# syshin1014/wssdl_bus

Measured on AMD Instinct MI355X. Metric: images/sec (train step, 600x1000), higher is better.
Workload: dtype f32; 1 GPU; resnet50_joint_b8; backbone=ResNet-50, image=600x1000, images_per_gpu=8, supervised_per_gpu=4, weak_per_gpu=4, mode=joint, parallelism=image-parallel dp1, RCCL grad all-reduce, sampling_rng=device, fused_rpn_softmax=True, padded_rois=False, miopen_find=True, miopen_find_db=wssdl_bus_amd/miopen_db (HIP.3_5_0_20250912-42-1199-g2584e35062), miopen_searched=True

## Files before the change

### wssdl_bus_amd/build.py

```python
import os
import subprocess
import sys

HERE = os.path.dirname(os.path.abspath(__file__))
CSRC = os.path.join(HERE, "csrc")
OUT = os.environ.get("WSSDL_BUS_HIP_LIB") or os.path.join(HERE, "libwssdl_bus_hip.so")
SOURCES = ["api_common.hip", "bbox_overlaps.hip", "nms.hip", "proposal.hip", "anchor_target.hip",
           "roi_targets.hip", "roi_pool.hip", "roi_pool_compact.hip", "roi_pool_blocks.hip", "roi_pool_walk.hip", "mil.hip", "image.hip", "loss.hip",
           "post_detect.hip", "order_sort.hip"]
HEADERS = ["common.hip.h", "nms.hip.h", "select.hip.h", "order_sort.hip.h", "roi_pool.hip.h", os.path.join("..", "..", "include", "wssdl_bus_hip.h")]
FLAGS = ["-O3", "-std=c++17", "--offload-arch=gfx950", "-ffp-contract=off", "-fPIC", "-shared",
         "-fvisibility=hidden", "-Wall", "-Wno-unused-function"]


def hipcc():
    for c in (os.environ.get("HIPCC"), "/opt/rocm/bin/hipcc", "hipcc"):
        if c and (os.path.isabs(c) and os.path.exists(c) or not os.path.isabs(c)):
            return c
    return "hipcc"


def is_stale():
    if not os.path.exists(OUT):
        return True
    t = os.path.getmtime(OUT)
    deps = [os.path.join(CSRC, s) for s in SOURCES + HEADERS] + [os.path.abspath(__file__), os.path.join(HERE, "isa_check.py")]
    return any(os.path.getmtime(d) > t for d in deps)


def _digest(paths, extra=""):
    import hashlib
    h = hashlib.sha256(extra.encode())
    for q in paths:
        with open(q, "rb") as f:
            h.update(f.read())
    return h.hexdigest()[:16]


def _compile_one(args):
    src, obj, flags, verbose = args
    tmp = "%s.%d.tmp" % (obj, os.getpid())
    cmd = [hipcc()] + flags + ["-c", src, "-o", tmp]
    if verbose:
        print("[wssdl_bus_amd] " + " ".join(cmd), flush=True)
    subprocess.check_call(cmd)
    os.replace(tmp, obj)
    return obj


def compile_objects(sources, headers, flags, verbose=True, jobs=None):
    from concurrent.futures import ThreadPoolExecutor
    objdir = os.path.join(CSRC, "_obj")
    os.makedirs(objdir, exist_ok=True)
    cflags = [f for f in flags if f != "-shared"]
    hdrs = [os.path.join(CSRC, h) for h in headers]
    todo, objs = [], []
    for s in sources:
        src = os.path.join(CSRC, s)
        tag = _digest([src] + hdrs, " ".join(cflags))
        obj = os.path.join(objdir, "%s.%s.o" % (os.path.basename(s), tag))
        objs.append(obj)
        if not os.path.exists(obj):
            for old in os.listdir(objdir):
                if old.startswith(os.path.basename(s) + "."):
                    os.remove(os.path.join(objdir, old))
            todo.append((src, obj, cflags, verbose))
    jobs = jobs or int(os.environ.get("WSSDL_BUILD_JOBS", "0")) or min(8, os.cpu_count() or 1)
    with ThreadPoolExecutor(max_workers=max(1, jobs)) as ex:
        list(ex.map(_compile_one, todo))
    return objs


def build(force=False, verbose=True):
    if not force and not is_stale():
        return OUT
    if force:
        import shutil
        shutil.rmtree(os.path.join(CSRC, "_obj"), ignore_errors=True)
    objs = compile_objects(SOURCES, HEADERS, FLAGS, verbose)
    tmp = "%s.%d.tmp" % (OUT, os.getpid())
    cmd = [hipcc(), "-shared", "-fPIC", "--offload-arch=gfx950", "-fvisibility=hidden"] + objs + ["-o", tmp]
    if verbose:
        print("[wssdl_bus_amd] " + " ".join(cmd))
    subprocess.check_call(cmd)
    from . import isa_check
    try:
        isa_check.check_library(tmp)
    except Exception:
        os.remove(tmp)
        raise
    os.replace(tmp, OUT)
    return OUT


PLUMB_OUT = os.path.join(HERE, "libwssdl_plumbing_hip.so")
PLUMB_SOURCES = [os.path.join("plumbing", "rowbn.hip"), os.path.join("plumbing", "im2col.hip")]
PLUMB_FLAGS = ["-O3", "-std=c++17", "--offload-arch=gfx950", "-fPIC", "-shared", "-fvisibility=hidden",
               "-Wall"]


def build_plumbing(force=False, verbose=True):
    srcs = [os.path.join(CSRC, s) for s in PLUMB_SOURCES]
    if not force and os.path.exists(PLUMB_OUT) and \
            all(os.path.getmtime(f) <= os.path.getmtime(PLUMB_OUT) for f in srcs + [os.path.abspath(__file__)]):
        return PLUMB_OUT
    tmp = "%s.%d.tmp" % (PLUMB_OUT, os.getpid())
    cmd = [hipcc()] + PLUMB_FLAGS + srcs + ["-o", tmp]
    if verbose:
        print("[wssdl_bus_amd] " + " ".join(cmd))
    subprocess.check_call(cmd)
    os.replace(tmp, PLUMB_OUT)
    return PLUMB_OUT


if __name__ == "__main__":
    build(force="--force" in sys.argv)
    build_plumbing(force="--force" in sys.argv)
    print(OUT)
    print(PLUMB_OUT)
```

### wssdl_bus_amd/csrc/plumbing/rowbn.hip

```cpp
#include <hip/hip_runtime.h>
#include <stdint.h>

#define PLUMB_API extern "C" __attribute__((visibility("default")))

namespace {

constexpr int BLOCK = 256;
constexpr int MAX_PARTIAL_BLOCKS = 1024;

typedef float float4v __attribute__((ext_vector_type(4)));

template <int MODE, bool RELU, bool MASKED>
__global__ __launch_bounds__(BLOCK) void rowbn_partial_kernel(
    const float *__restrict__ x, const float *__restrict__ dy, const float *__restrict__ scale,
    const float *__restrict__ shift, long long M, int C, long long rows_per_block,
    double *__restrict__ partial, const float *__restrict__ mask, int per) {
    __shared__ double red[BLOCK][8];
    const int C4 = C >> 2;
    const int L = C4 < BLOCK ? C4 : BLOCK;
    const int RS = BLOCK / L;
    const int t = threadIdx.x;
    const int lc = t % L, lr = t / L;
    const long long r0 = (long long)blockIdx.x * rows_per_block;
    const long long r1 = r0 + rows_per_block < M ? r0 + rows_per_block : M;
    double *out = partial + (size_t)blockIdx.x * 2 * C;
    for (int cc = 0; cc * L < C4; ++cc) {
        const int c4 = cc * L + lc;
        double s[4] = {0, 0, 0, 0}, q[4] = {0, 0, 0, 0};
        float4v sc = {0, 0, 0, 0}, sh = {0, 0, 0, 0};
        if (MODE == 1 && RELU) {
            sc = reinterpret_cast<const float4v *>(scale)[c4];
            sh = reinterpret_cast<const float4v *>(shift)[c4];
        }
        if (lr < RS) {
            long long r = r0 + lr;
            for (; r + RS < r1; r += 2 * RS) {
                bool live0 = true, live1 = true;
                if (MASKED) {
                    live0 = mask[(unsigned)r / (unsigned)per] != 0.0f;
                    live1 = mask[(unsigned)(r + RS) / (unsigned)per] != 0.0f;
                    if (!live0 && !live1) continue;
                }
                const float4v zero4 = {0, 0, 0, 0};
                const float4v a0 = live0 ? reinterpret_cast<const float4v *>(x + (size_t)r * C)[c4] : zero4;
                const float4v a1 = live1 ? reinterpret_cast<const float4v *>(x + (size_t)(r + RS) * C)[c4] : zero4;
                float4v g0, g1;
                if (MODE == 1) {
                    g0 = live0 ? reinterpret_cast<const float4v *>(dy + (size_t)r * C)[c4] : zero4;
                    g1 = live1 ? reinterpret_cast<const float4v *>(dy + (size_t)(r + RS) * C)[c4] : zero4;
                }
#pragma unroll
                for (int j = 0; j < 4; ++j) {
                    if (MODE == 0) {
                        s[j] += (double)a0[j] + (double)a1[j];
                        q[j] += (double)a0[j] * (double)a0[j] + (double)a1[j] * (double)a1[j];
                    } else {
                        float u0 = g0[j], u1 = g1[j];
                        if (RELU) {
                            if (!(a0[j] * sc[j] + sh[j] > 0.0f)) u0 = 0.0f;
                            if (!(a1[j] * sc[j] + sh[j] > 0.0f)) u1 = 0.0f;
                        }
                        if (MASKED) {
                            if (!live0) u0 = 0.0f;
                            if (!live1) u1 = 0.0f;
                        }
                        s[j] += (double)u0 + (double)u1;
                        q[j] += (double)u0 * (double)a0[j] + (double)u1 * (double)a1[j];
                    }
                }
            }
            for (; r < r1; r += RS) {
                if (MASKED && mask[(unsigned)r / (unsigned)per] == 0.0f) continue;
                const float4v a0 = reinterpret_cast<const float4v *>(x + (size_t)r * C)[c4];
                float4v g0;
                if (MODE == 1) g0 = reinterpret_cast<const float4v *>(dy + (size_t)r * C)[c4];
#pragma unroll
                for (int j = 0; j < 4; ++j) {
                    if (MODE == 0) {
                        s[j] += (double)a0[j];
                        q[j] += (double)a0[j] * (double)a0[j];
                    } else {
                        float u0 = g0[j];
                        if (RELU && !(a0[j] * sc[j] + sh[j] > 0.0f)) u0 = 0.0f;
                        s[j] += (double)u0;
                        q[j] += (double)u0 * (double)a0[j];
                    }
                }
            }
        }
        __syncthreads();
#pragma unroll
        for (int j = 0; j < 4; ++j) { red[t][j] = s[j]; red[t][4 + j] = q[j]; }
        __syncthreads();
        if (lr == 0) {
#pragma unroll
            for (int j = 0; j < 4; ++j) {
                double ss = 0.0, qq = 0.0;
                for (int k = 0; k < RS; ++k) { ss += red[k * L + lc][j]; qq += red[k * L + lc][4 + j]; }
                out[c4 * 4 + j] = ss;
                out[C + c4 * 4 + j] = qq;
            }
        }
    }
}

constexpr int FIN_COLS = 16, FIN_GROUPS = 64;

__device__ __forceinline__ void finish_reduce(const double *__restrict__ partial, int nblocks, int C,
                                              int c, int grp, double (*red)[FIN_COLS][2], double &s,
                                              double &q) {
    double ss = 0.0, qq = 0.0;
    if (c < C)
        for (int b = grp; b < nblocks; b += FIN_GROUPS) {
            ss += partial[(size_t)b * 2 * C + c];
            qq += partial[(size_t)b * 2 * C + C + c];
        }
    red[grp][threadIdx.x % FIN_COLS][0] = ss;
    red[grp][threadIdx.x % FIN_COLS][1] = qq;
    __syncthreads();
    s = 0.0;
    q = 0.0;
    if (grp == 0)
        for (int g = 0; g < FIN_GROUPS; ++g) {
            s += red[g][threadIdx.x][0];
            q += red[g][threadIdx.x][1];
        }
}

__device__ __forceinline__ double live_rows(const float *__restrict__ mask, int n_rois, int per, long long M,
                                            double *scratch ) {
    if (!mask) return (double)M;
    double c = 0.0;
    for (int i = threadIdx.x; i < n_rois; i += FIN_COLS * FIN_GROUPS) c += mask[i] != 0.0f ? 1.0 : 0.0;
    __syncthreads();
    scratch[threadIdx.x] = c;
    __syncthreads();
    double t = 0.0;
    for (int i = 0; i < FIN_COLS * FIN_GROUPS; ++i) t += scratch[i];
    __syncthreads();
    t *= (double)per;
    return t < 1.0 ? 1.0 : t;
}

__global__ __launch_bounds__(FIN_COLS * FIN_GROUPS) void rowbn_fwd_finish_kernel(
    const double *__restrict__ partial, int nblocks, int C, long long M,
    const float *__restrict__ weight, const float *__restrict__ bias, float eps,
    float *__restrict__ mean, float *__restrict__ var, float *__restrict__ rstd,
    float *__restrict__ scale, float *__restrict__ shift, const float *__restrict__ mask, int n_rois, int per,
    float *__restrict__ count) {
    __shared__ double red[FIN_GROUPS][FIN_COLS][2];
    const int grp = threadIdx.x / FIN_COLS;
    const int c = blockIdx.x * FIN_COLS + threadIdx.x % FIN_COLS;
    const double Mn = live_rows(mask, n_rois, per, M, &red[0][0][0]);
    if (count && blockIdx.x == 0 && threadIdx.x == 0) count[0] = (float)Mn;
    double s, q;
    finish_reduce(partial, nblocks, C, c, grp, red, s, q);
    if (grp != 0 || c >= C) return;
    const double mu = s / Mn;
    double v = q / Mn - mu * mu;
    if (v < 0.0) v = 0.0;
    const float rs = (float)(1.0 / sqrt(v + (double)eps));
    const float scl = rs * weight[c];
    mean[c] = (float)mu;
    var[c] = (float)v;
    rstd[c] = rs;
    scale[c] = scl;
    shift[c] = bias[c] - (float)mu * scl;
}

__global__ __launch_bounds__(FIN_COLS * FIN_GROUPS) void rowbn_bwd_finish_kernel(
    const double *__restrict__ partial, int nblocks, int C, long long M,
    const float *__restrict__ weight, const float *__restrict__ mean,
    const float *__restrict__ rstd, float *__restrict__ dweight, float *__restrict__ dbias,
    float *__restrict__ coef, const float *__restrict__ mask, int n_rois, int per) {
    __shared__ double red[FIN_GROUPS][FIN_COLS][2];
    const int grp = threadIdx.x / FIN_COLS;
    const int c = blockIdx.x * FIN_COLS + threadIdx.x % FIN_COLS;
    const double Mn = live_rows(mask, n_rois, per, M, &red[0][0][0]);
    double sg, sgx;
    finish_reduce(partial, nblocks, C, c, grp, red, sg, sgx);
    if (grp != 0 || c >= C) return;
    const double mu = mean[c], rs = rstd[c], w = weight[c];
    const double sum_g_xhat = (sgx - mu * sg) * rs;
    const double a = w * rs;
    const double k1 = a * rs * sum_g_xhat / Mn;
    const double k0 = a * sg / Mn - k1 * mu;
    dweight[c] = (float)sum_g_xhat;
    dbias[c] = (float)sg;
    coef[c] = (float)a;
    coef[C + c] = (float)k0;
    coef[2 * C + c] = (float)k1;
}

template <bool RELU, bool MASKED>
__global__ __launch_bounds__(BLOCK) void rowbn_apply_fwd_kernel(
    const float *__restrict__ x, const float *__restrict__ scale, const float *__restrict__ shift,
    long long total4, int C4, float *__restrict__ y, const float *__restrict__ mask, int per) {
    for (long long i = (long long)blockIdx.x * BLOCK + threadIdx.x; i < total4;
         i += (long long)gridDim.x * BLOCK) {
        const int c4 = (int)(i % C4);
        if (MASKED && mask[(unsigned)(i / C4) / (unsigned)per] == 0.0f) {
            const float4v zero4 = {0, 0, 0, 0};
            reinterpret_cast<float4v *>(y)[i] = zero4;
            continue;
        }
        const float4v a = reinterpret_cast<const float4v *>(x)[i];
        const float4v sc = reinterpret_cast<const float4v *>(scale)[c4];
        const float4v sh = reinterpret_cast<const float4v *>(shift)[c4];
        float4v o;
#pragma unroll
        for (int j = 0; j < 4; ++j) {
            float v = a[j] * sc[j] + sh[j];
            if (RELU) v = v > 0.0f ? v : 0.0f;
            o[j] = v;
        }
        reinterpret_cast<float4v *>(y)[i] = o;
    }
}

template <bool RELU, bool MASKED>
__global__ __launch_bounds__(BLOCK) void rowbn_apply_bwd_kernel(
    const float *__restrict__ x, const float *__restrict__ dy, const float *__restrict__ scale,
    const float *__restrict__ shift, const float *__restrict__ coef, long long total4, int C4,
    float *__restrict__ dx, const float *__restrict__ mask, int per) {
    const int C = C4 * 4;
    for (long long i = (long long)blockIdx.x * BLOCK + threadIdx.x; i < total4;
         i += (long long)gridDim.x * BLOCK) {
        const int c4 = (int)(i % C4);
        if (MASKED && mask[(unsigned)(i / C4) / (unsigned)per] == 0.0f) {
            const float4v zero4 = {0, 0, 0, 0};
            reinterpret_cast<float4v *>(dx)[i] = zero4;
            continue;
        }
        const float4v a = reinterpret_cast<const float4v *>(x)[i];
        const float4v g = reinterpret_cast<const float4v *>(dy)[i];
        const float4v ka = reinterpret_cast<const float4v *>(coef)[c4];
        const float4v k0 = reinterpret_cast<const float4v *>(coef + C)[c4];
        const float4v k1 = reinterpret_cast<const float4v *>(coef + 2 * C)[c4];
        float4v sc = {0, 0, 0, 0}, sh = {0, 0, 0, 0};
        if (RELU) {
            sc = reinterpret_cast<const float4v *>(scale)[c4];
            sh = reinterpret_cast<const float4v *>(shift)[c4];
        }
        float4v o;
#pragma unroll
        for (int j = 0; j < 4; ++j) {
            float u = g[j];
            if (RELU && !(a[j] * sc[j] + sh[j] > 0.0f)) u = 0.0f;
            o[j] = ka[j] * u - k0[j] - k1[j] * a[j];
        }
        reinterpret_cast<float4v *>(dx)[i] = o;
    }
}

inline int partial_blocks(long long M, int C) {
    const int C4 = C / 4;
    const int L = C4 < BLOCK ? C4 : BLOCK;
    const int RS = BLOCK / L;
    long long want = (M + (long long)RS * 16 - 1) / ((long long)RS * 16);
    if (want < 1) want = 1;
    return (int)(want < MAX_PARTIAL_BLOCKS ? want : MAX_PARTIAL_BLOCKS);
}

inline bool shape_ok(long long M, int C) {
    if (M < 1 || C < 4 || (C & 3)) return false;
    const int C4 = C / 4;
    return C4 <= BLOCK ? (BLOCK % C4 == 0) : (C4 % BLOCK == 0);
}

inline int apply_grid(long long total4) {
    long long b = (total4 + BLOCK - 1) / BLOCK;
    return (int)(b < 65536 ? b : 65536);
}

}

PLUMB_API size_t wsplumb_rowbn_workspace_bytes(long long M, int C) {
    if (!shape_ok(M, C)) return 0;
    return (size_t)partial_blocks(M, C) * 2 * (size_t)C * sizeof(double);
}

PLUMB_API int wsplumb_rowbn_supported(long long M, int C) { return shape_ok(M, C) ? 1 : 0; }

static int forward_impl(const float *x, long long M, int C, const float *weight, const float *bias, float eps,
                        int relu, float *y, float *mean, float *var, float *rstd, float *scale, float *shift,
                        const float *mask, int n_rois, int per, float *count, void *workspace,
                        size_t workspace_bytes, void *stream) {
    if (!shape_ok(M, C) || workspace_bytes < wsplumb_rowbn_workspace_bytes(M, C)) return 1;
    if (mask && (per < 1 || n_rois < 1 || (long long)n_rois * per != M || M > 0x7fffffffLL)) return 1;
    hipStream_t st = static_cast<hipStream_t>(stream);
    const int nb = partial_blocks(M, C);
    const long long rpb = (M + nb - 1) / nb;
    double *partial = static_cast<double *>(workspace);
    if (mask)
        hipLaunchKernelGGL((rowbn_partial_kernel<0, false, true>), dim3(nb), dim3(BLOCK), 0, st, x, nullptr,
                           nullptr, nullptr, M, C, rpb, partial, mask, per);
    else
        hipLaunchKernelGGL((rowbn_partial_kernel<0, false, false>), dim3(nb), dim3(BLOCK), 0, st, x, nullptr,
                           nullptr, nullptr, M, C, rpb, partial, nullptr, 1);
    hipLaunchKernelGGL(rowbn_fwd_finish_kernel, dim3((C + FIN_COLS - 1) / FIN_COLS), dim3(FIN_COLS * FIN_GROUPS), 0, st, partial, nb, C,
                       M, weight, bias, eps, mean, var, rstd, scale, shift, mask, n_rois, per, count);
    const long long total4 = M * (C / 4);
#define WSPLUMB_APPLY(RELU, MASKED) \
    hipLaunchKernelGGL((rowbn_apply_fwd_kernel<RELU, MASKED>), dim3(apply_grid(total4)), dim3(BLOCK), 0, st, x, scale, \
                       shift, total4, C / 4, y, mask, per)
    if (relu) { if (mask) WSPLUMB_APPLY(true, true); else WSPLUMB_APPLY(true, false); }
    else { if (mask) WSPLUMB_APPLY(false, true); else WSPLUMB_APPLY(false, false); }
#undef WSPLUMB_APPLY
    return hipGetLastError() == hipSuccess ? 0 : 3;
}

PLUMB_API int wsplumb_rowbn_forward(const float *x, long long M, int C, const float *weight,
                                    const float *bias, float eps, int relu, float *y, float *mean,
                                    float *var, float *rstd, float *scale, float *shift,
                                    void *workspace, size_t workspace_bytes, void *stream) {
    return forward_impl(x, M, C, weight, bias, eps, relu, y, mean, var, rstd, scale, shift, nullptr, 0, 1, nullptr,
                        workspace, workspace_bytes, stream);
}

PLUMB_API int wsplumb_rowbn_forward_masked(const float *x, long long M, int C, const float *weight,
                                           const float *bias, float eps, int relu, const float *mask,
                                           int n_rois, int per, float *y, float *mean, float *var,
                                           float *rstd, float *scale, float *shift, float *count,
                                           void *workspace, size_t workspace_bytes, void *stream) {
    if (!mask || !count) return 1;
    return forward_impl(x, M, C, weight, bias, eps, relu, y, mean, var, rstd, scale, shift, mask, n_rois, per, count,
                        workspace, workspace_bytes, stream);
}

PLUMB_API int wsplumb_rowbn_apply(const float *x, long long M, int C, const float *scale,
                                  const float *shift, int relu, float *y, void *stream) {
    if (M < 1 || C < 4 || (C & 3)) return 1;
    hipStream_t st = static_cast<hipStream_t>(stream);
    const long long total4 = M * (C / 4);
    if (relu)
        hipLaunchKernelGGL((rowbn_apply_fwd_kernel<true, false>), dim3(apply_grid(total4)), dim3(BLOCK), 0, st, x,
                           scale, shift, total4, C / 4, y, nullptr, 1);
    else
        hipLaunchKernelGGL((rowbn_apply_fwd_kernel<false, false>), dim3(apply_grid(total4)), dim3(BLOCK), 0, st, x,
                           scale, shift, total4, C / 4, y, nullptr, 1);
    return hipGetLastError() == hipSuccess ? 0 : 3;
}

static int backward_impl(const float *x, const float *dy, long long M, int C, const float *weight,
                         const float *mean, const float *rstd, const float *scale, const float *shift, int relu,
                         float *dx, float *dweight, float *dbias, float *coef, const float *mask, int n_rois,
                         int per, void *workspace, size_t workspace_bytes, void *stream) {
    if (!shape_ok(M, C) || workspace_bytes < wsplumb_rowbn_workspace_bytes(M, C)) return 1;
    if (mask && (per < 1 || n_rois < 1 || (long long)n_rois * per != M || M > 0x7fffffffLL)) return 1;
    hipStream_t st = static_cast<hipStream_t>(stream);
    const int nb = partial_blocks(M, C);
    const long long rpb = (M + nb - 1) / nb;
    double *partial = static_cast<double *>(workspace);
#define WSPLUMB_PARTIAL(RELU, MASKED) \
    hipLaunchKernelGGL((rowbn_partial_kernel<1, RELU, MASKED>), dim3(nb), dim3(BLOCK), 0, st, x, dy, scale, shift, M, C, \
                       rpb, partial, mask, per)
    if (relu) { if (mask) WSPLUMB_PARTIAL(true, true); else WSPLUMB_PARTIAL(true, false); }
    else { if (mask) WSPLUMB_PARTIAL(false, true); else WSPLUMB_PARTIAL(false, false); }
#undef WSPLUMB_PARTIAL
    hipLaunchKernelGGL(rowbn_bwd_finish_kernel, dim3((C + FIN_COLS - 1) / FIN_COLS), dim3(FIN_COLS * FIN_GROUPS), 0, st, partial, nb, C,
                       M, weight, mean, rstd, dweight, dbias, coef, mask, n_rois, per);
    const long long total4 = M * (C / 4);
#define WSPLUMB_APPLY(RELU, MASKED) \
    hipLaunchKernelGGL((rowbn_apply_bwd_kernel<RELU, MASKED>), dim3(apply_grid(total4)), dim3(BLOCK), 0, st, x, dy, scale, \
                       shift, coef, total4, C / 4, dx, mask, per)
    if (relu) { if (mask) WSPLUMB_APPLY(true, true); else WSPLUMB_APPLY(true, false); }
    else { if (mask) WSPLUMB_APPLY(false, true); else WSPLUMB_APPLY(false, false); }
#undef WSPLUMB_APPLY
    return hipGetLastError() == hipSuccess ? 0 : 3;
}

PLUMB_API int wsplumb_rowbn_backward(const float *x, const float *dy, long long M, int C,
                                     const float *weight, const float *mean, const float *rstd,
                                     const float *scale, const float *shift, int relu, float *dx,
                                     float *dweight, float *dbias, float *coef, void *workspace,
                                     size_t workspace_bytes, void *stream) {
    return backward_impl(x, dy, M, C, weight, mean, rstd, scale, shift, relu, dx, dweight, dbias, coef, nullptr, 0, 1,
                         workspace, workspace_bytes, stream);
}

PLUMB_API int wsplumb_rowbn_backward_masked(const float *x, const float *dy, long long M, int C,
                                            const float *weight, const float *mean, const float *rstd,
                                            const float *scale, const float *shift, int relu,
                                            const float *mask, int n_rois, int per, float *dx,
                                            float *dweight, float *dbias, float *coef, void *workspace,
                                            size_t workspace_bytes, void *stream) {
    if (!mask) return 1;
    return backward_impl(x, dy, M, C, weight, mean, rstd, scale, shift, relu, dx, dweight, dbias, coef, mask, n_rois, per,
                         workspace, workspace_bytes, stream);
}
```

### wssdl_bus_amd/networks/_plumbing.py

```python
import ctypes
import os
import warnings

import torch

_HERE = os.path.dirname(os.path.dirname(os.path.abspath(__file__)))
LIB_PATH = os.path.join(_HERE, "libwssdl_plumbing_hip.so")
_lib = None
_warned = [False]

_vp, _i, _ll, _f, _sz = ctypes.c_void_p, ctypes.c_int, ctypes.c_longlong, ctypes.c_float, ctypes.c_size_t


def lib():
    global _lib
    if _lib is None:
        if not os.path.exists(LIB_PATH):
            if not _warned[0]:
                _warned[0] = True
                warnings.warn("%s not built: the per-RoI head uses stock PyTorch batch-norm ops "
                              "(python -m wssdl_bus_amd.build builds it)" % LIB_PATH)
            return None
        L = ctypes.CDLL(LIB_PATH)
        L.wsplumb_rowbn_workspace_bytes.restype = _sz
        L.wsplumb_rowbn_workspace_bytes.argtypes = [_ll, _i]
        L.wsplumb_rowbn_supported.restype = _i
        L.wsplumb_rowbn_supported.argtypes = [_ll, _i]
        L.wsplumb_rowbn_forward.restype = _i
        L.wsplumb_rowbn_forward.argtypes = [_vp, _ll, _i, _vp, _vp, _f, _i, _vp, _vp, _vp, _vp, _vp, _vp,
                                            _vp, _sz, _vp]
        L.wsplumb_rowbn_apply.restype = _i
        L.wsplumb_rowbn_apply.argtypes = [_vp, _ll, _i, _vp, _vp, _i, _vp, _vp]
        L.wsplumb_rowbn_backward.restype = _i
        L.wsplumb_rowbn_backward.argtypes = [_vp, _vp, _ll, _i, _vp, _vp, _vp, _vp, _vp, _i, _vp, _vp, _vp,
                                             _vp, _vp, _sz, _vp]
        L.wsplumb_rowbn_forward_masked.restype = _i
        L.wsplumb_rowbn_forward_masked.argtypes = [_vp, _ll, _i, _vp, _vp, _f, _i, _vp, _i, _i, _vp, _vp, _vp, _vp,
                                                   _vp, _vp, _vp, _vp, _sz, _vp]
        L.wsplumb_rowbn_backward_masked.restype = _i
        L.wsplumb_rowbn_backward_masked.argtypes = [_vp, _vp, _ll, _i, _vp, _vp, _vp, _vp, _vp, _i, _vp, _i, _i,
                                                    _vp, _vp, _vp, _vp, _vp, _sz, _vp]
        for name in ("wsplumb_im2col3x3", "wsplumb_col2im3x3"):
            f = getattr(L, name)
            f.restype = _i
            f.argtypes = [_vp, _ll, _i, _i, _i, _i, _i, _i, _i, _i, _vp, _vp]
        _lib = L
    return _lib


def _p(t):
    return ctypes.c_void_p(t.data_ptr())


def _stream():
    return ctypes.c_void_p(torch.cuda.current_stream().cuda_stream)


def usable(x):
    if os.environ.get("WSSDL_DISABLE_FUSED_BN"):
        return False
    if not (x.is_cuda and x.dtype == torch.float32 and x.dim() == 2 and x.is_contiguous()):
        return False
    L = lib()
    return L is not None and bool(L.wsplumb_rowbn_supported(x.shape[0], x.shape[1]))


def _workspace(L, M, C, dev):
    n = L.wsplumb_rowbn_workspace_bytes(M, C)
    return torch.empty((n,), dtype=torch.uint8, device=dev), n


def rowbn_forward(x, weight, bias, eps, relu, mask=None):
    L = lib()
    M, C = x.shape
    dev = x.device
    y = torch.empty_like(x)
    stats = torch.empty((5, C), dtype=torch.float32, device=dev)
    count = None
    with torch.cuda.device(dev):
        ws, n = _workspace(L, M, C, dev)
        if mask is None:
            rc = L.wsplumb_rowbn_forward(_p(x), M, C, _p(weight), _p(bias), float(eps), int(relu), _p(y),
                                         _p(stats[0]), _p(stats[1]), _p(stats[2]), _p(stats[3]),
                                         _p(stats[4]), _p(ws), n, _stream())
        else:
            n_rois = mask.shape[0]
            assert M % n_rois == 0 and mask.dtype == torch.float32 and mask.is_contiguous()
            count = torch.empty((1,), dtype=torch.float32, device=dev)
            rc = L.wsplumb_rowbn_forward_masked(_p(x), M, C, _p(weight), _p(bias), float(eps), int(relu), _p(mask),
                                                n_rois, M // n_rois, _p(y), _p(stats[0]), _p(stats[1]), _p(stats[2]),
                                                _p(stats[3]), _p(stats[4]), _p(count), _p(ws), n, _stream())
    if rc:
        raise RuntimeError("wsplumb_rowbn_forward failed (%d)" % rc)
    return y, stats, count


def rowbn_apply(x, scale, shift, relu):
    L = lib()
    M, C = x.shape
    y = torch.empty_like(x)
    with torch.cuda.device(x.device):
        rc = L.wsplumb_rowbn_apply(_p(x), M, C, _p(scale), _p(shift), int(relu), _p(y), _stream())
    if rc:
        raise RuntimeError("wsplumb_rowbn_apply failed (%d)" % rc)
    return y


def rowbn_backward(x, dy, weight, stats, relu, mask=None):
    L = lib()
    M, C = x.shape
    dev = x.device
    dx = torch.empty_like(x)
    dwb = torch.empty((2, C), dtype=torch.float32, device=dev)
    coef = torch.empty((3, C), dtype=torch.float32, device=dev)
    with torch.cuda.device(dev):
        ws, n = _workspace(L, M, C, dev)
        if mask is None:
            rc = L.wsplumb_rowbn_backward(_p(x), _p(dy), M, C, _p(weight), _p(stats[0]), _p(stats[2]),
                                          _p(stats[3]), _p(stats[4]), int(relu), _p(dx), _p(dwb[0]),
                                          _p(dwb[1]), _p(coef), _p(ws), n, _stream())
        else:
            n_rois = mask.shape[0]
            rc = L.wsplumb_rowbn_backward_masked(_p(x), _p(dy), M, C, _p(weight), _p(stats[0]), _p(stats[2]),
                                                 _p(stats[3]), _p(stats[4]), int(relu), _p(mask), n_rois,
                                                 M // n_rois, _p(dx), _p(dwb[0]), _p(dwb[1]), _p(coef), _p(ws), n,
                                                 _stream())
    if rc:
        raise RuntimeError("wsplumb_rowbn_backward failed (%d)" % rc)
    return dx, dwb[0], dwb[1]


def im2col_usable(x):
    if os.environ.get("WSSDL_DISABLE_FUSED_IM2COL"):
        return False
    return (x.is_cuda and x.dtype == torch.float32 and x.dim() == 4 and x.is_contiguous()
            and x.shape[3] % 4 == 0 and x.shape[0] > 0 and lib() is not None)


class Im2Col3x3Fn(torch.autograd.Function):

    @staticmethod
    def forward(ctx, x, stride, oh, ow, pt, pl):
        L = lib()
        r, h, w, c = x.shape
        cols = torch.empty((r * oh * ow, 9 * c), dtype=torch.float32, device=x.device)
        with torch.cuda.device(x.device):
            rc = L.wsplumb_im2col3x3(_p(x), r, h, w, c, oh, ow, stride, pt, pl, _p(cols), _stream())
        if rc:
            raise RuntimeError("wsplumb_im2col3x3 failed (%d)" % rc)
        ctx.geom = (r, h, w, c, oh, ow, stride, pt, pl)
        return cols

    @staticmethod
    def backward(ctx, dcols):
        L = lib()
        r, h, w, c, oh, ow, stride, pt, pl = ctx.geom
        dcols = dcols.contiguous()
        dx = torch.empty((r, h, w, c), dtype=torch.float32, device=dcols.device)
        with torch.cuda.device(dcols.device):
            rc = L.wsplumb_col2im3x3(_p(dcols), r, h, w, c, oh, ow, stride, pt, pl, _p(dx), _stream())
        if rc:
            raise RuntimeError("wsplumb_col2im3x3 failed (%d)" % rc)
        return dx, None, None, None, None, None
```

### wssdl_bus_amd/networks/roi_head.py

```python
import torch
import torch.nn as nn
import torch.nn.functional as F

from . import _plumbing
from .backbones import RESNET_DEFS, _same_pad


class _RowBatchNormFn(torch.autograd.Function):

    @staticmethod
    def forward(ctx, x, weight, bias, eps):
        var, mean = torch.var_mean(x, dim=0, unbiased=False)
        rstd = torch.rsqrt(var + eps)
        scale = rstd * weight
        y = torch.addcmul(bias - mean * scale, x, scale)
        ctx.save_for_backward(x, mean, rstd, weight)
        ctx.mark_non_differentiable(mean, var)
        return y, mean, var

    @staticmethod
    def backward(ctx, dy, _dmean, _dvar):
        x, mean, rstd, weight = ctx.saved_tensors
        m = x.shape[0]
        sum_dy = dy.sum(0)
        sum_dy_x = (dy * x).sum(0)
        sum_dy_xhat = (sum_dy_x - mean * sum_dy) * rstd
        a = weight * rstd
        k1 = a * rstd * sum_dy_xhat / m
        k0 = a * sum_dy / m - k1 * mean
        dx = torch.addcmul(-k0, dy, a)
        dx.addcmul_(x, -k1)
        return dx, sum_dy_xhat, sum_dy, None


class _FusedRowBatchNormFn(torch.autograd.Function):

    @staticmethod
    def forward(ctx, x, weight, bias, eps, relu, roi_mask=None):
        y, stats, count = _plumbing.rowbn_forward(x, weight, bias, eps, relu, roi_mask)
        ctx.masked = roi_mask is not None
        if ctx.masked:
            ctx.save_for_backward(x, weight, stats, roi_mask)
        else:
            ctx.save_for_backward(x, weight, stats)
            count = stats[0, :1]
        ctx.relu = relu
        mean, var = stats[0], stats[1]
        ctx.mark_non_differentiable(mean, var, count)
        return y, mean, var, count

    @staticmethod
    def backward(ctx, dy, _dmean, _dvar, _dcount):
        if ctx.masked:
            x, weight, stats, roi_mask = ctx.saved_tensors
        else:
            (x, weight, stats), roi_mask = ctx.saved_tensors, None
        dx, dw, db = _plumbing.rowbn_backward(x, dy.contiguous(), weight, stats, ctx.relu, roi_mask)
        return dx, dw, db, None, None, None


_ROI_MASK = None


def set_roi_mask(mask):
    global _ROI_MASK
    _ROI_MASK = mask


def _masked_row_batch_norm(x, weight, bias, eps, relu, roi_mask):
    M = x.shape[0]
    per = M // roi_mask.shape[0]
    m = roi_mask.repeat_interleave(per).unsqueeze(1)
    n = (roi_mask.sum() * per).clamp_min(1.0)
    mean = (x * m).sum(0) / n
    d = (x - mean) * m
    var = (d * d).sum(0) / n
    y = d * (torch.rsqrt(var + eps) * weight) + bias
    if relu:
        y = F.relu(y)
    return y * m, mean.detach(), var.detach(), n


class RowBatchNorm(nn.Module):

    def __init__(self, num_features, eps=1e-3, momentum=0.01):
        super().__init__()
        self.eps, self.momentum = eps, momentum
        self.weight = nn.Parameter(torch.ones(num_features))
        self.bias = nn.Parameter(torch.zeros(num_features))
        self.register_buffer("running_mean", torch.zeros(num_features))
        self.register_buffer("running_var", torch.ones(num_features))

    def forward(self, x, relu=False):
        fused = _plumbing.usable(x)
        if not self.training:
            scale = self.weight * torch.rsqrt(self.running_var + self.eps)
            shift = self.bias - self.running_mean * scale
            if fused and not torch.is_grad_enabled():
                return _plumbing.rowbn_apply(x, scale.contiguous(), shift.contiguous(), relu)
            y = torch.addcmul(shift, x, scale)
            return F.relu(y) if relu else y
        if _ROI_MASK is not None:
            if fused and x.shape[0] % _ROI_MASK.shape[0] == 0:
                y, mean, var, n = _FusedRowBatchNormFn.apply(x, self.weight, self.bias, self.eps, bool(relu), _ROI_MASK)
                n = n[0]
            else:
                y, mean, var, n = _masked_row_batch_norm(x, self.weight, self.bias, self.eps, relu, _ROI_MASK)
            with torch.no_grad():
                self.running_mean.lerp_(mean, self.momentum)
                self.running_var.lerp_(var * (n / (n - 1).clamp_min(1.0)), self.momentum)
            return y
        if fused:
            y, mean, var, _ = _FusedRowBatchNormFn.apply(x, self.weight, self.bias, self.eps, bool(relu))
        else:
            y, mean, var = _RowBatchNormFn.apply(x, self.weight, self.bias, self.eps)
            if relu:
                y = F.relu(y)
        with torch.no_grad():
            m = x.shape[0]
            self.running_mean.lerp_(mean, self.momentum)
            self.running_var.lerp_(var * (m / max(m - 1, 1)), self.momentum)
        return y


class ConvNHWC(nn.Module):

    def __init__(self, c_i, c_o, k, s, norm=None, relu=True):
        super().__init__()
        self.c_i, self.c_o, self.k, self.s, self.relu = c_i, c_o, k, s, relu
        self.weight = nn.Parameter(torch.empty(c_o, k * k * c_i))
        nn.init.trunc_normal_(self.weight, std=0.01, a=-0.02, b=0.02)
        self.bias = nn.Parameter(torch.zeros(c_o)) if norm is None else None
        self.bn = RowBatchNorm(c_o) if norm == "BN" else None

    def forward(self, x):
        r, h, w, c = x.shape
        k, s = self.k, self.s
        if k == 1:
            if s > 1:
                x = x[:, ::s, ::s, :]
            oh, ow = x.shape[1], x.shape[2]
            rows = x.reshape(-1, c)
        elif k == 3 and _plumbing.im2col_usable(x):
            pt, pb = _same_pad(h, k, s)
            pl, pr = _same_pad(w, k, s)
            oh, ow = -(-h // s), -(-w // s)
            rows = _plumbing.Im2Col3x3Fn.apply(x, s, oh, ow, pt, pl)
        else:
            pt, pb = _same_pad(h, k, s)
            pl, pr = _same_pad(w, k, s)
            xp = F.pad(x, (0, 0, pl, pr, pt, pb))
            p = xp.unfold(1, k, s).unfold(2, k, s)
            oh, ow = p.shape[1], p.shape[2]
            rows = p.permute(0, 1, 2, 4, 5, 3).reshape(-1, k * k * c)
        y = F.linear(rows, self.weight, self.bias)
        if self.bn is not None:
            y = self.bn(y, relu=self.relu)
        elif self.relu:
            y = F.relu(y)
        return y.view(r, oh, ow, self.c_o)


def _bn_rows(bn, x, relu=False):
    r, h, w, c = x.shape
    return bn(x.reshape(-1, c), relu=relu).view(r, h, w, c)


class BottleneckNHWC(nn.Module):
    expansion = 4

    def __init__(self, c_i, c_o, s, preact, norm):
        super().__init__()
        self.preact = preact
        self.pre_bn = RowBatchNorm(c_i) if (preact != "no_preact" and norm == "BN") else None
        self.conv1 = ConvNHWC(c_i, c_o, 1, 1, norm)
        self.conv2 = ConvNHWC(c_o, c_o, 3, s, norm)
        self.conv3 = ConvNHWC(c_o, c_o * 4, 1, 1, norm, relu=False)
        self.short = ConvNHWC(c_i, c_o * 4, 1, s, norm, relu=False) if c_i != c_o * 4 else None

    def forward(self, x):
        ori = x
        if self.preact != "no_preact":
            y = _bn_rows(self.pre_bn, x, relu=True) if self.pre_bn is not None else F.relu(x)
            if self.preact == "both_preact":
                ori = y
            x = y
        x = self.conv3(self.conv2(self.conv1(x)))
        return x + (self.short(ori) if self.short is not None else ori)


class BasicBlockNHWC(nn.Module):
    expansion = 1

    def __init__(self, c_i, c_o, s, preact, norm):
        super().__init__()
        self.preact = preact
        self.pre_bn = RowBatchNorm(c_i) if (preact != "no_preact" and norm == "BN") else None
        self.conv1 = ConvNHWC(c_i, c_o, 3, s, norm)
        self.conv2 = ConvNHWC(c_o, c_o, 3, 1, norm, relu=False)
        self.short = ConvNHWC(c_i, c_o, 1, s, norm, relu=False) if c_i != c_o else None

    def forward(self, x):
        ori = x
        if self.preact != "no_preact":
            y = _bn_rows(self.pre_bn, x, relu=True) if self.pre_bn is not None else F.relu(x)
            if self.preact == "both_preact":
                ori = y
            x = y
        x = self.conv2(self.conv1(x))
        return x + (self.short(ori) if self.short is not None else ori)


class ResNetHeadNHWC(nn.Module):

    def __init__(self, depth, norm="BN"):
        super().__init__()
        defs, block = RESNET_DEFS[depth]
        blk = BottleneckNHWC if block.expansion == 4 else BasicBlockNHWC
        e = blk.expansion
        blocks = [blk(256 * e, 512, 2, "both_preact", norm)]
        for _ in range(1, defs[3]):
            blocks.append(blk(512 * e, 512, 1, "default", norm))
        self.group3 = nn.Sequential(*blocks)
        self.norm = RowBatchNorm(512 * e) if norm == "BN" else None
        self.out_features = 512 * e

    def forward(self, x):
        x = self.group3(x)
        x = _bn_rows(self.norm, x, relu=True) if self.norm is not None else F.relu(x)
        return x.mean(dim=(1, 2))
```

Before: 48.84 images/s.

## Run ROI head in position-major layout with tap-grouped 3x3 convolutions

Adds a position-major execution path for the ResNet ROI head. Rows are ordered by spatial position and then ROI, and 3x3 convs become tap-class gathers plus batched GEMMs that group positions sharing the same valid kernel taps, so padded taps are skipped. RowBatchNorm gains a pos-major mask mode (modulo instead of divide) so the masked BN kernels work on the new layout. The cost is extra gather/col2im and weight-scatter kernels, more small GEMM launches and planning complexity, and it falls back to the old path when the plan is not usable.

```diff
diff --git a/wssdl_bus_amd/build.py b/wssdl_bus_amd/build.py
--- a/wssdl_bus_amd/build.py
+++ b/wssdl_bus_amd/build.py
@@ -94,7 +94,8 @@
 
 
 PLUMB_OUT = os.path.join(HERE, "libwssdl_plumbing_hip.so")
-PLUMB_SOURCES = [os.path.join("plumbing", "rowbn.hip"), os.path.join("plumbing", "im2col.hip")]
+PLUMB_SOURCES = [os.path.join("plumbing", "rowbn.hip"), os.path.join("plumbing", "im2col.hip"),
+                 os.path.join("plumbing", "taps.hip")]
 PLUMB_FLAGS = ["-O3", "-std=c++17", "--offload-arch=gfx950", "-fPIC", "-shared", "-fvisibility=hidden",
                "-Wall"]
 
diff --git a/wssdl_bus_amd/csrc/plumbing/rowbn.hip b/wssdl_bus_amd/csrc/plumbing/rowbn.hip
--- a/wssdl_bus_amd/csrc/plumbing/rowbn.hip
+++ b/wssdl_bus_amd/csrc/plumbing/rowbn.hip
@@ -10,7 +10,12 @@
 
 typedef float float4v __attribute__((ext_vector_type(4)));
 
-template <int MODE, bool RELU, bool MASKED>
+template <int MASK>
+__device__ __forceinline__ unsigned mask_roi(long long r, int div) {
+    return MASK == 2 ? (unsigned)r % (unsigned)div : (unsigned)r / (unsigned)div;
+}
+
+template <int MODE, bool RELU, int MASK>
 __global__ __launch_bounds__(BLOCK) void rowbn_partial_kernel(
     const float *__restrict__ x, const float *__restrict__ dy, const float *__restrict__ scale,
     const float *__restrict__ shift, long long M, int C, long long rows_per_block,
@@ -36,9 +41,9 @@
             long long r = r0 + lr;
             for (; r + RS < r1; r += 2 * RS) {
                 bool live0 = true, live1 = true;
-                if (MASKED) {
-                    live0 = mask[(unsigned)r / (unsigned)per] != 0.0f;
-                    live1 = mask[(unsigned)(r + RS) / (unsigned)per] != 0.0f;
+                if (MASK) {
+                    live0 = mask[mask_roi<MASK>(r, per)] != 0.0f;
+                    live1 = mask[mask_roi<MASK>(r + RS, per)] != 0.0f;
                     if (!live0 && !live1) continue;
                 }
                 const float4v zero4 = {0, 0, 0, 0};
@@ -60,7 +65,7 @@
                             if (!(a0[j] * sc[j] + sh[j] > 0.0f)) u0 = 0.0f;
                             if (!(a1[j] * sc[j] + sh[j] > 0.0f)) u1 = 0.0f;
                         }
-                        if (MASKED) {
+                        if (MASK) {
                             if (!live0) u0 = 0.0f;
                             if (!live1) u1 = 0.0f;
                         }
@@ -70,7 +75,7 @@
                 }
             }
             for (; r < r1; r += RS) {
-                if (MASKED && mask[(unsigned)r / (unsigned)per] == 0.0f) continue;
+                if (MASK && mask[mask_roi<MASK>(r, per)] == 0.0f) continue;
                 const float4v a0 = reinterpret_cast<const float4v *>(x + (size_t)r * C)[c4];
                 float4v g0;
                 if (MODE == 1) g0 = reinterpret_cast<const float4v *>(dy + (size_t)r * C)[c4];
@@ -192,14 +197,14 @@
     coef[2 * C + c] = (float)k1;
 }
 
-template <bool RELU, bool MASKED>
+template <bool RELU, int MASK>
 __global__ __launch_bounds__(BLOCK) void rowbn_apply_fwd_kernel(
     const float *__restrict__ x, const float *__restrict__ scale, const float *__restrict__ shift,
     long long total4, int C4, float *__restrict__ y, const float *__restrict__ mask, int per) {
     for (long long i = (long long)blockIdx.x * BLOCK + threadIdx.x; i < total4;
          i += (long long)gridDim.x * BLOCK) {
         const int c4 = (int)(i % C4);
-        if (MASKED && mask[(unsigned)(i / C4) / (unsigned)per] == 0.0f) {
+        if (MASK && mask[mask_roi<MASK>(i / C4, per)] == 0.0f) {
             const float4v zero4 = {0, 0, 0, 0};
             reinterpret_cast<float4v *>(y)[i] = zero4;
             continue;
@@ -218,7 +223,7 @@
     }
 }
 
-template <bool RELU, bool MASKED>
+template <bool RELU, int MASK>
 __global__ __launch_bounds__(BLOCK) void rowbn_apply_bwd_kernel(
     const float *__restrict__ x, const float *__restrict__ dy, const float *__restrict__ scale,
     const float *__restrict__ shift, const float *__restrict__ coef, long long total4, int C4,
@@ -227,7 +232,7 @@
     for (long long i = (long long)blockIdx.x * BLOCK + threadIdx.x; i < total4;
          i += (long long)gridDim.x * BLOCK) {
         const int c4 = (int)(i % C4);
-        if (MASKED && mask[(unsigned)(i / C4) / (unsigned)per] == 0.0f) {
+        if (MASK && mask[mask_roi<MASK>(i / C4, per)] == 0.0f) {
             const float4v zero4 = {0, 0, 0, 0};
             reinterpret_cast<float4v *>(dx)[i] = zero4;
             continue;
@@ -285,27 +290,32 @@
 static int forward_impl(const float *x, long long M, int C, const float *weight, const float *bias, float eps,
                         int relu, float *y, float *mean, float *var, float *rstd, float *scale, float *shift,
                         const float *mask, int n_rois, int per, float *count, void *workspace,
-                        size_t workspace_bytes, void *stream) {
+                        size_t workspace_bytes, void *stream, bool pm = false) {
     if (!shape_ok(M, C) || workspace_bytes < wsplumb_rowbn_workspace_bytes(M, C)) return 1;
     if (mask && (per < 1 || n_rois < 1 || (long long)n_rois * per != M || M > 0x7fffffffLL)) return 1;
     hipStream_t st = static_cast<hipStream_t>(stream);
     const int nb = partial_blocks(M, C);
     const long long rpb = (M + nb - 1) / nb;
     double *partial = static_cast<double *>(workspace);
-    if (mask)
-        hipLaunchKernelGGL((rowbn_partial_kernel<0, false, true>), dim3(nb), dim3(BLOCK), 0, st, x, nullptr,
+    const int div = pm ? n_rois : per;
+    if (mask && pm)
+        hipLaunchKernelGGL((rowbn_partial_kernel<0, false, 2>), dim3(nb), dim3(BLOCK), 0, st, x, nullptr,
+                           nullptr, nullptr, M, C, rpb, partial, mask, div);
+    else if (mask)
+        hipLaunchKernelGGL((rowbn_partial_kernel<0, false, 1>), dim3(nb), dim3(BLOCK), 0, st, x, nullptr,
                            nullptr, nullptr, M, C, rpb, partial, mask, per);
     else
-        hipLaunchKernelGGL((rowbn_partial_kernel<0, false, false>), dim3(nb), dim3(BLOCK), 0, st, x, nullptr,
+        hipLaunchKernelGGL((rowbn_partial_kernel<0, false, 0>), dim3(nb), dim3(BLOCK), 0, st, x, nullptr,
                            nullptr, nullptr, M, C, rpb, partial, nullptr, 1);
     hipLaunchKernelGGL(rowbn_fwd_finish_kernel, dim3((C + FIN_COLS - 1) / FIN_COLS), dim3(FIN_COLS * FIN_GROUPS), 0, st, partial, nb, C,
                        M, weight, bias, eps, mean, var, rstd, scale, shift, mask, n_rois, per, count);
     const long long total4 = M * (C / 4);
-#define WSPLUMB_APPLY(RELU, MASKED) \
-    hipLaunchKernelGGL((rowbn_apply_fwd_kernel<RELU, MASKED>), dim3(apply_grid(total4)), dim3(BLOCK), 0, st, x, scale, \
-                       shift, total4, C / 4, y, mask, per)
-    if (relu) { if (mask) WSPLUMB_APPLY(true, true); else WSPLUMB_APPLY(true, false); }
-    else { if (mask) WSPLUMB_APPLY(false, true); else WSPLUMB_APPLY(false, false); }
+#define WSPLUMB_APPLY(RELU, MASK) \
+    hipLaunchKernelGGL((rowbn_apply_fwd_kernel<RELU, MASK>), dim3(apply_grid(total4)), dim3(BLOCK), 0, st, x, scale, \
+                       shift, total4, C / 4, y, mask, div)
+    const int mode = mask ? (pm ? 2 : 1) : 0;
+    if (relu) { if (mode == 2) WSPLUMB_APPLY(true, 2); else if (mode) WSPLUMB_APPLY(true, 1); else WSPLUMB_APPLY(true, 0); }
+    else { if (mode == 2) WSPLUMB_APPLY(false, 2); else if (mode) WSPLUMB_APPLY(false, 1); else WSPLUMB_APPLY(false, 0); }
 #undef WSPLUMB_APPLY
     return hipGetLastError() == hipSuccess ? 0 : 3;
 }
@@ -334,10 +344,10 @@
     hipStream_t st = static_cast<hipStream_t>(stream);
     const long long total4 = M * (C / 4);
     if (relu)
-        hipLaunchKernelGGL((rowbn_apply_fwd_kernel<true, false>), dim3(apply_grid(total4)), dim3(BLOCK), 0, st, x,
+        hipLaunchKernelGGL((rowbn_apply_fwd_kernel<true, 0>), dim3(apply_grid(total4)), dim3(BLOCK), 0, st, x,
                            scale, shift, total4, C / 4, y, nullptr, 1);
     else
-        hipLaunchKernelGGL((rowbn_apply_fwd_kernel<false, false>), dim3(apply_grid(total4)), dim3(BLOCK), 0, st, x,
+        hipLaunchKernelGGL((rowbn_apply_fwd_kernel<false, 0>), dim3(apply_grid(total4)), dim3(BLOCK), 0, st, x,
                            scale, shift, total4, C / 4, y, nullptr, 1);
     return hipGetLastError() == hipSuccess ? 0 : 3;
 }
@@ -345,27 +355,29 @@
 static int backward_impl(const float *x, const float *dy, long long M, int C, const float *weight,
                          const float *mean, const float *rstd, const float *scale, const float *shift, int relu,
                          float *dx, float *dweight, float *dbias, float *coef, const float *mask, int n_rois,
-                         int per, void *workspace, size_t workspace_bytes, void *stream) {
+                         int per, void *workspace, size_t workspace_bytes, void *stream, bool pm = false) {
     if (!shape_ok(M, C) || workspace_bytes < wsplumb_rowbn_workspace_bytes(M, C)) return 1;
     if (mask && (per < 1 || n_rois < 1 || (long long)n_rois * per != M || M > 0x7fffffffLL)) return 1;
     hipStream_t st = static_cast<hipStream_t>(stream);
     const int nb = partial_blocks(M, C);
     const long long rpb = (M + nb - 1) / nb;
     double *partial = static_cast<double *>(workspace);
-#define WSPLUMB_PARTIAL(RELU, MASKED) \
-    hipLaunchKernelGGL((rowbn_partial_kernel<1, RELU, MASKED>), dim3(nb), dim3(BLOCK), 0, st, x, dy, scale, shift, M, C, \
-                       rpb, partial, mask, per)
-    if (relu) { if (mask) WSPLUMB_PARTIAL(true, true); else WSPLUMB_PARTIAL(true, false); }
-    else { if (mask) WSPLUMB_PARTIAL(false, true); else WSPLUMB_PARTIAL(false, false); }
+    const int div = pm ? n_rois : per;
+    const int mode = mask ? (pm ? 2 : 1) : 0;
+#define WSPLUMB_PARTIAL(RELU, MASK) \
+    hipLaunchKernelGGL((rowbn_partial_kernel<1, RELU, MASK>), dim3(nb), dim3(BLOCK), 0, st, x, dy, scale, shift, M, C, \
+                       rpb, partial, mask, div)
+    if (relu) { if (mode == 2) WSPLUMB_PARTIAL(true, 2); else if (mode) WSPLUMB_PARTIAL(true, 1); else WSPLUMB_PARTIAL(true, 0); }
+    else { if (mode == 2) WSPLUMB_PARTIAL(false, 2); else if (mode) WSPLUMB_PARTIAL(false, 1); else WSPLUMB_PARTIAL(false, 0); }
 #undef WSPLUMB_PARTIAL
     hipLaunchKernelGGL(rowbn_bwd_finish_kernel, dim3((C + FIN_COLS - 1) / FIN_COLS), dim3(FIN_COLS * FIN_GROUPS), 0, st, partial, nb, C,
                        M, weight, mean, rstd, dweight, dbias, coef, mask, n_rois, per);
     const long long total4 = M * (C / 4);
-#define WSPLUMB_APPLY(RELU, MASKED) \
-    hipLaunchKernelGGL((rowbn_apply_bwd_kernel<RELU, MASKED>), dim3(apply_grid(total4)), dim3(BLOCK), 0, st, x, dy, scale, \
-                       shift, coef, total4, C / 4, dx, mask, per)
-    if (relu) { if (mask) WSPLUMB_APPLY(true, true); else WSPLUMB_APPLY(true, false); }
-    else { if (mask) WSPLUMB_APPLY(false, true); else WSPLUMB_APPLY(false, false); }
+#define WSPLUMB_APPLY(RELU, MASK) \
+    hipLaunchKernelGGL((rowbn_apply_bwd_kernel<RELU, MASK>), dim3(apply_grid(total4)), dim3(BLOCK), 0, st, x, dy, scale, \
+                       shift, coef, total4, C / 4, dx, mask, div)
+    if (relu) { if (mode == 2) WSPLUMB_APPLY(true, 2); else if (mode) WSPLUMB_APPLY(true, 1); else WSPLUMB_APPLY(true, 0); }
+    else { if (mode == 2) WSPLUMB_APPLY(false, 2); else if (mode) WSPLUMB_APPLY(false, 1); else WSPLUMB_APPLY(false, 0); }
 #undef WSPLUMB_APPLY
     return hipGetLastError() == hipSuccess ? 0 : 3;
 }
@@ -389,3 +401,24 @@
     return backward_impl(x, dy, M, C, weight, mean, rstd, scale, shift, relu, dx, dweight, dbias, coef, mask, n_rois, per,
                          workspace, workspace_bytes, stream);
 }
+
+PLUMB_API int wsplumb_rowbn_forward_masked_pm(const float *x, long long M, int C, const float *weight,
+                                              const float *bias, float eps, int relu, const float *mask,
+                                              int n_rois, int per, float *y, float *mean, float *var,
+                                              float *rstd, float *scale, float *shift, float *count,
+                                              void *workspace, size_t workspace_bytes, void *stream) {
+    if (!mask || !count) return 1;
+    return forward_impl(x, M, C, weight, bias, eps, relu, y, mean, var, rstd, scale, shift, mask, n_rois, per, count,
+                        workspace, workspace_bytes, stream, true);
+}
+
+PLUMB_API int wsplumb_rowbn_backward_masked_pm(const float *x, const float *dy, long long M, int C,
+                                               const float *weight, const float *mean, const float *rstd,
+                                               const float *scale, const float *shift, int relu,
+                                               const float *mask, int n_rois, int per, float *dx,
+                                               float *dweight, float *dbias, float *coef, void *workspace,
+                                               size_t workspace_bytes, void *stream) {
+    if (!mask) return 1;
+    return backward_impl(x, dy, M, C, weight, mean, rstd, scale, shift, relu, dx, dweight, dbias, coef, mask, n_rois, per,
+                         workspace, workspace_bytes, stream, true);
+}
diff --git a/wssdl_bus_amd/csrc/plumbing/taps.hip b/wssdl_bus_amd/csrc/plumbing/taps.hip
--- /dev/null
+++ b/wssdl_bus_amd/csrc/plumbing/taps.hip
@@ -0,0 +1,192 @@
+#include <hip/hip_runtime.h>
+#include <stdint.h>
+
+#define PLUMB_API extern "C" __attribute__((visibility("default")))
+
+namespace {
+
+constexpr int TAB_NCLS = 0, TAB_H = 1, TAB_W = 2, TAB_OH = 3, TAB_OW = 4, TAB_S = 5, TAB_PT = 6, TAB_PL = 7,
+              TAB_UNITS = 8, TAB_WUNITS = 9;
+constexpr int TAB_CLS = 16, CLS_STRIDE = 24, MAX_CLS = 9;
+constexpr int C_NPOS = 0, C_NTAPS = 1, C_SLOT = 2, C_CUM = 3, C_WCUM = 4,
+              C_TAPS = 6,
+              C_TAPIDX = 15;
+constexpr int MAX_POS = 64;
+constexpr int TAB_SLOTPOS = TAB_CLS + CLS_STRIDE * MAX_CLS;
+constexpr int TAB_POSSLOT = TAB_SLOTPOS + MAX_POS;
+constexpr int TAB_SLOTCLS = TAB_POSSLOT + MAX_POS;
+constexpr int TAB_INTS = TAB_SLOTCLS + MAX_POS;
+
+typedef float float4v __attribute__((ext_vector_type(4)));
+
+__device__ __forceinline__ const int *cls_of(const int *T, int k) { return T + TAB_CLS + CLS_STRIDE * k; }
+
+template <int F>
+__device__ __forceinline__ int find_class(const int *__restrict__ T, unsigned q) {
+    const int n = T[TAB_NCLS];
+    int k = 0;
+    while (k + 1 < n && (unsigned)cls_of(T, k + 1)[F] <= q) ++k;
+    return k;
+}
+
+__global__ __launch_bounds__(256) void tap_gather_kernel(const float *__restrict__ x, const int *__restrict__ T,
+                                                        int in_pm, unsigned R, unsigned C4, unsigned total4,
+                                                        float *__restrict__ cols) {
+    const int H = T[TAB_H], W = T[TAB_W], OW = T[TAB_OW], S = T[TAB_S], PT = T[TAB_PT], PL = T[TAB_PL];
+    const unsigned unit4 = R * C4;
+    for (unsigned i = blockIdx.x * 256u + threadIdx.x; i < total4; i += gridDim.x * 256u) {
+        const int k = find_class<C_CUM>(T, i / unit4);
+        const int *cl = cls_of(T, k);
+        const unsigned ntaps = cl[C_NTAPS];
+        const unsigned local = i - (unsigned)cl[C_CUM] * unit4;
+        const unsigned c4 = local % C4, t = local / C4;
+        const unsigned tl = t % ntaps, row = t / ntaps;
+        const unsigned roi = row % R, p = row / R;
+        const int pos = T[TAB_SLOTPOS + cl[C_SLOT] + p];
+        const int tap = cl[C_TAPS + tl];
+        const int y = (pos / OW) * S + tap / 3 - PT, xx = (pos % OW) * S + tap % 3 - PL;
+        float4v v = {0.f, 0.f, 0.f, 0.f};
+        if (y >= 0 && y < H && xx >= 0 && xx < W) {
+            const size_t src = in_pm ? (size_t)T[TAB_POSSLOT + y * W + xx] * R + roi
+                                     : ((size_t)roi * H + y) * W + xx;
+            v = reinterpret_cast<const float4v *>(x)[src * C4 + c4];
+        }
+        reinterpret_cast<float4v *>(cols)[i] = v;
+    }
+}
+
+__global__ __launch_bounds__(256) void tap_col2im_kernel(const float *__restrict__ dcols, const int *__restrict__ T,
+                                                        int in_pm, unsigned R, unsigned C4, unsigned total4,
+                                                        float *__restrict__ dx) {
+    const int H = T[TAB_H], W = T[TAB_W], OH = T[TAB_OH], OW = T[TAB_OW], S = T[TAB_S], PT = T[TAB_PT],
+              PL = T[TAB_PL];
+    const unsigned unit4 = R * C4;
+    for (unsigned i = blockIdx.x * 256u + threadIdx.x; i < total4; i += gridDim.x * 256u) {
+        const unsigned c4 = i % C4, row = i / C4;
+        unsigned roi;
+        int y, xx;
+        if (in_pm) {
+            roi = row % R;
+            const int pos = T[TAB_SLOTPOS + row / R];
+            y = pos / W;
+            xx = pos % W;
+        } else {
+            xx = (int)(row % (unsigned)W);
+            const unsigned t = row / (unsigned)W;
+            y = (int)(t % (unsigned)H);
+            roi = t / (unsigned)H;
+        }
+        float4v acc = {0.f, 0.f, 0.f, 0.f};
+#pragma unroll
+        for (int ky = 0; ky < 3; ++ky) {
+            const int ny = y + PT - ky;
+            if (ny < 0 || ny % S != 0) continue;
+            const int oy = ny / S;
+            if (oy >= OH) continue;
+#pragma unroll
+            for (int kx = 0; kx < 3; ++kx) {
+                const int nx = xx + PL - kx;
+                if (nx < 0 || nx % S != 0) continue;
+                const int ox = nx / S;
+                if (ox >= OW) continue;
+                const int slot = T[TAB_POSSLOT + oy * OW + ox];
+                const int *cl = cls_of(T, T[TAB_SLOTCLS + slot]);
+                const int tl = cl[C_TAPIDX + ky * 3 + kx];
+                if (tl < 0) continue;
+                const size_t u = (size_t)cl[C_CUM] * unit4 +
+                                 (((size_t)(slot - cl[C_SLOT]) * R + roi) * cl[C_NTAPS] + tl) * C4 + c4;
+                acc += reinterpret_cast<const float4v *>(dcols)[u];
+            }
+        }
+        reinterpret_cast<float4v *>(dx)[i] = acc;
+    }
+}
+
+__global__ __launch_bounds__(256) void tap_weight_gather_kernel(const float *__restrict__ w, const int *__restrict__ T,
+                                                               unsigned CO, unsigned C4, unsigned total4,
+                                                               float *__restrict__ wp) {
+    const unsigned unit4 = CO * C4;
+    for (unsigned i = blockIdx.x * 256u + threadIdx.x; i < total4; i += gridDim.x * 256u) {
+        const int k = find_class<C_WCUM>(T, i / unit4);
+        const int *cl = cls_of(T, k);
+        const unsigned ntaps = cl[C_NTAPS];
+        const unsigned local = i - (unsigned)cl[C_WCUM] * unit4;
+        const unsigned c4 = local % C4, t = local / C4;
+        const unsigned tl = t % ntaps, o = t / ntaps;
+        reinterpret_cast<float4v *>(wp)[i] =
+            reinterpret_cast<const float4v *>(w)[((size_t)o * 9 + cl[C_TAPS + tl]) * C4 + c4];
+    }
+}
+
+__global__ __launch_bounds__(256) void tap_weight_scatter_kernel(const float *__restrict__ dwp, const int *__restrict__ T,
+                                                                unsigned CO, unsigned C4, unsigned total4,
+                                                                float *__restrict__ dw) {
+    const int n = T[TAB_NCLS];
+    const unsigned unit4 = CO * C4;
+    for (unsigned i = blockIdx.x * 256u + threadIdx.x; i < total4; i += gridDim.x * 256u) {
+        const unsigned c4 = i % C4, t = i / C4;
+        const unsigned tap = t % 9u, o = t / 9u;
+        float4v acc = {0.f, 0.f, 0.f, 0.f};
+        for (int k = 0; k < n; ++k) {
+            const int *cl = cls_of(T, k);
+            const int tl = cl[C_TAPIDX + tap];
+            if (tl < 0) continue;
+            acc += reinterpret_cast<const float4v *>(dwp)[(size_t)cl[C_WCUM] * unit4 +
+                                                           ((size_t)o * cl[C_NTAPS] + tl) * C4 + c4];
+        }
+        reinterpret_cast<float4v *>(dw)[i] = acc;
+    }
+}
+
+inline int grid_for(unsigned total4) {
+    unsigned b = (total4 + 255u) / 256u;
+    return (int)(b < 262144u ? b : 262144u);
+}
+
+inline bool dims_ok(long long R, int C, long long total4) {
+    return R >= 1 && C >= 4 && !(C & 3) && total4 >= 1 && total4 <= 0x7fffffffLL;
+}
+
+}
+
+PLUMB_API int wsplumb_tap_table_ints() { return TAB_INTS; }
+
+PLUMB_API int wsplumb_tap_gather(const float *x, long long R, int C, const int *tab, const int *hnum, int in_pm,
+                                 float *cols, void *stream) {
+    const long long total4 = (long long)hnum[TAB_UNITS] * R * (C / 4);
+    if (R < 1 || C < 4 || (C & 3)) return 1;
+    if (!dims_ok(R, C, total4) || (long long)hnum[TAB_H] * hnum[TAB_W] * R * (C / 4) > 0x7fffffffLL) return 2;
+    hipLaunchKernelGGL(tap_gather_kernel, dim3(grid_for((unsigned)total4)), dim3(256), 0,
+                       static_cast<hipStream_t>(stream), x, tab, in_pm, (unsigned)R, (unsigned)(C / 4),
+                       (unsigned)total4, cols);
+    return hipGetLastError() == hipSuccess ? 0 : 3;
+}
+
+PLUMB_API int wsplumb_tap_col2im(const float *dcols, long long R, int C, const int *tab, const int *hnum, int in_pm,
+                                 float *dx, void *stream) {
+    const long long total4 = (long long)hnum[TAB_H] * hnum[TAB_W] * R * (C / 4);
+    if (R < 1 || C < 4 || (C & 3)) return 1;
+    if (!dims_ok(R, C, total4) || (long long)hnum[TAB_UNITS] * R * (C / 4) > 0x7fffffffLL) return 2;
+    hipLaunchKernelGGL(tap_col2im_kernel, dim3(grid_for((unsigned)total4)), dim3(256), 0,
+                       static_cast<hipStream_t>(stream), dcols, tab, in_pm, (unsigned)R, (unsigned)(C / 4),
+                       (unsigned)total4, dx);
+    return hipGetLastError() == hipSuccess ? 0 : 3;
+}
+
+PLUMB_API int wsplumb_tap_weight_gather(const float *w, int CO, int C, const int *tab, const int *hnum, float *wp,
+                                        void *stream) {
+    const long long total4 = (long long)hnum[TAB_WUNITS] * CO * (C / 4);
+    if (CO < 1 || !dims_ok(CO, C, total4) || 9LL * CO * (C / 4) > 0x7fffffffLL) return 1;
+    hipLaunchKernelGGL(tap_weight_gather_kernel, dim3(grid_for((unsigned)total4)), dim3(256), 0,
+                       static_cast<hipStream_t>(stream), w, tab, (unsigned)CO, (unsigned)(C / 4), (unsigned)total4, wp);
+    return hipGetLastError() == hipSuccess ? 0 : 3;
+}
+
+PLUMB_API int wsplumb_tap_weight_scatter(const float *dwp, int CO, int C, const int *tab, const int *hnum, float *dw,
+                                         void *stream) {
+    const long long total4 = 9LL * CO * (C / 4);
+    if (CO < 1 || !dims_ok(CO, C, total4) || (long long)hnum[TAB_WUNITS] * CO * (C / 4) > 0x7fffffffLL) return 1;
+    hipLaunchKernelGGL(tap_weight_scatter_kernel, dim3(grid_for((unsigned)total4)), dim3(256), 0,
+                       static_cast<hipStream_t>(stream), dwp, tab, (unsigned)CO, (unsigned)(C / 4), (unsigned)total4, dw);
+    return hipGetLastError() == hipSuccess ? 0 : 3;
+}
diff --git a/wssdl_bus_amd/networks/_plumbing.py b/wssdl_bus_amd/networks/_plumbing.py
--- a/wssdl_bus_amd/networks/_plumbing.py
+++ b/wssdl_bus_amd/networks/_plumbing.py
@@ -40,6 +40,19 @@
         L.wsplumb_rowbn_backward_masked.restype = _i
         L.wsplumb_rowbn_backward_masked.argtypes = [_vp, _vp, _ll, _i, _vp, _vp, _vp, _vp, _vp, _i, _vp, _i, _i,
                                                     _vp, _vp, _vp, _vp, _vp, _sz, _vp]
+        for name in ("wsplumb_rowbn_forward_masked_pm", "wsplumb_rowbn_backward_masked_pm"):
+            base = getattr(L, name[:-3])
+            getattr(L, name).restype, getattr(L, name).argtypes = base.restype, base.argtypes
+        L.wsplumb_tap_table_ints.restype = _i
+        L.wsplumb_tap_table_ints.argtypes = []
+        for name in ("wsplumb_tap_gather", "wsplumb_tap_col2im"):
+            f = getattr(L, name)
+            f.restype = _i
+            f.argtypes = [_vp, _ll, _i, _vp, _vp, _i, _vp, _vp]
+        for name in ("wsplumb_tap_weight_gather", "wsplumb_tap_weight_scatter"):
+            f = getattr(L, name)
+            f.restype = _i
+            f.argtypes = [_vp, _i, _i, _vp, _vp, _vp, _vp]
         for name in ("wsplumb_im2col3x3", "wsplumb_col2im3x3"):
             f = getattr(L, name)
             f.restype = _i
@@ -70,7 +83,7 @@
     return torch.empty((n,), dtype=torch.uint8, device=dev), n
 
 
-def rowbn_forward(x, weight, bias, eps, relu, mask=None):
+def rowbn_forward(x, weight, bias, eps, relu, mask=None, pos_major=False):
     L = lib()
     M, C = x.shape
     dev = x.device
@@ -87,9 +100,10 @@
             n_rois = mask.shape[0]
             assert M % n_rois == 0 and mask.dtype == torch.float32 and mask.is_contiguous()
             count = torch.empty((1,), dtype=torch.float32, device=dev)
-            rc = L.wsplumb_rowbn_forward_masked(_p(x), M, C, _p(weight), _p(bias), float(eps), int(relu), _p(mask),
-                                                n_rois, M // n_rois, _p(y), _p(stats[0]), _p(stats[1]), _p(stats[2]),
-                                                _p(stats[3]), _p(stats[4]), _p(count), _p(ws), n, _stream())
+            fn = L.wsplumb_rowbn_forward_masked_pm if pos_major else L.wsplumb_rowbn_forward_masked
+            rc = fn(_p(x), M, C, _p(weight), _p(bias), float(eps), int(relu), _p(mask), n_rois, M // n_rois, _p(y),
+                    _p(stats[0]), _p(stats[1]), _p(stats[2]), _p(stats[3]), _p(stats[4]), _p(count), _p(ws), n,
+                    _stream())
     if rc:
         raise RuntimeError("wsplumb_rowbn_forward failed (%d)" % rc)
     return y, stats, count
@@ -106,7 +120,7 @@
     return y
 
 
-def rowbn_backward(x, dy, weight, stats, relu, mask=None):
+def rowbn_backward(x, dy, weight, stats, relu, mask=None, pos_major=False):
     L = lib()
     M, C = x.shape
     dev = x.device
@@ -121,10 +135,9 @@
                                           _p(dwb[1]), _p(coef), _p(ws), n, _stream())
         else:
             n_rois = mask.shape[0]
-            rc = L.wsplumb_rowbn_backward_masked(_p(x), _p(dy), M, C, _p(weight), _p(stats[0]), _p(stats[2]),
-                                                 _p(stats[3]), _p(stats[4]), int(relu), _p(mask), n_rois,
-                                                 M // n_rois, _p(dx), _p(dwb[0]), _p(dwb[1]), _p(coef), _p(ws), n,
-                                                 _stream())
+            fn = L.wsplumb_rowbn_backward_masked_pm if pos_major else L.wsplumb_rowbn_backward_masked
+            rc = fn(_p(x), _p(dy), M, C, _p(weight), _p(stats[0]), _p(stats[2]), _p(stats[3]), _p(stats[4]), int(relu),
+                    _p(mask), n_rois, M // n_rois, _p(dx), _p(dwb[0]), _p(dwb[1]), _p(coef), _p(ws), n, _stream())
     if rc:
         raise RuntimeError("wsplumb_rowbn_backward failed (%d)" % rc)
     return dx, dwb[0], dwb[1]
@@ -162,3 +175,218 @@
         if rc:
             raise RuntimeError("wsplumb_col2im3x3 failed (%d)" % rc)
         return dx, None, None, None, None, None
+
+
+_TAB_CLS, _CLS_STRIDE, _MAX_CLS, _MAX_POS = 16, 24, 9, 64
+_TAB_SLOTPOS = _TAB_CLS + _CLS_STRIDE * _MAX_CLS
+_TAB_POSSLOT, _TAB_SLOTCLS = _TAB_SLOTPOS + _MAX_POS, _TAB_SLOTPOS + 2 * _MAX_POS
+_TAB_INTS = _TAB_SLOTCLS + _MAX_POS
+
+TAP_GEMM_GROUPED = True
+TAPS_MIN_ROIS = 2048
+
+
+class TapPlan:
+
+    def __init__(self, h, w, s):
+        from .backbones import _same_pad
+        self.h, self.w, self.s = h, w, s
+        self.pt, self.pl = _same_pad(h, 3, s)[0], _same_pad(w, 3, s)[0]
+        self.oh, self.ow = -(-h // s), -(-w // s)
+
+        def axis(n_in, n_out, pad):
+            cls = {}
+            for o in range(n_out):
+                taps = tuple(k for k in range(3) if 0 <= o * s + k - pad < n_in)
+                cls.setdefault(taps, []).append(o)
+            return list(cls.items())
+
+        classes = []
+        for ty, ys in axis(h, self.oh, self.pt):
+            for tx, xs in axis(w, self.ow, self.pl):
+                classes.append(([ky * 3 + kx for ky in ty for kx in tx], [(y, x) for y in ys for x in xs]))
+        classes.sort(key=lambda c: (-len(c[0]), -len(c[1])))
+        self.classes = classes
+        self.slots = [p for _, pos in classes for p in pos]
+        self.groups, k = [], 0
+        while k < len(classes):
+            j = k
+            while j < len(classes) and (len(classes[j][0]), len(classes[j][1])) == \
+                    (len(classes[k][0]), len(classes[k][1])):
+                j += 1
+            self.groups.append((k, j - k, len(classes[k][1]), len(classes[k][0])))
+            k = j
+        self.cum, self.wcum, self.slot_base = [], [], []
+        u = wu = sb = 0
+        for taps, pos in classes:
+            self.cum.append(u)
+            self.wcum.append(wu)
+            self.slot_base.append(sb)
+            u, wu, sb = u + len(taps) * len(pos), wu + len(taps), sb + len(pos)
+        self.units, self.wunits = u, wu
+        self.ok = (len(classes) <= _MAX_CLS and self.oh * self.ow <= _MAX_POS and h * w <= _MAX_POS
+                   and self.units < 9 * self.oh * self.ow)
+        self.table = self._table()
+        self.hnum = self.table.ctypes.data_as(ctypes.c_void_p)
+        self._dev = {}
+
+    def _table(self):
+        import numpy as np
+        T = np.full(_TAB_INTS, -1, np.int32)
+        T[:10] = [len(self.classes), self.h, self.w, self.oh, self.ow, self.s, self.pt, self.pl, self.units,
+                  self.wunits]
+        for k, (taps, pos) in enumerate(self.classes[:_MAX_CLS]):
+            b = _TAB_CLS + _CLS_STRIDE * k
+            T[b:b + 5] = [len(pos), len(taps), self.slot_base[k], self.cum[k], self.wcum[k]]
+            T[b + 6:b + 6 + len(taps)] = taps
+            for i, t in enumerate(taps):
+                T[b + 15 + t] = i
+        for sl, (y, x) in enumerate(self.slots[:_MAX_POS]):
+            T[_TAB_SLOTPOS + sl] = y * self.ow + x
+            T[_TAB_POSSLOT + y * self.ow + x] = sl
+            T[_TAB_SLOTCLS + sl] = next(k for k in range(len(self.classes))
+                                        if self.slot_base[k] <= sl < self.slot_base[k] + len(self.classes[k][1]))
+        return T
+
+    def device_table(self, dev):
+        t = self._dev.get(dev)
+        if t is None:
+            t = self._dev[dev] = torch.from_numpy(self.table).to(dev)
+        return t
+
+    def subsample_index(self, w_in, s, dev):
+        key = ("sub", w_in, s, dev)
+        t = self._dev.get(key)
+        if t is None:
+            t = self._dev[key] = torch.tensor([y * s * w_in + x * s for y, x in self.slots],
+                                              dtype=torch.long, device=dev)
+        return t
+
+
+_PLANS = {}
+
+
+def tap_plan(h, w, s):
+    p = _PLANS.get((h, w, s))
+    if p is None:
+        p = _PLANS[(h, w, s)] = TapPlan(h, w, s)
+    return p
+
+
+def taps_usable(x):
+    if os.environ.get("WSSDL_HEAD_DENSE_3X3"):
+        return False
+    return im2col_usable(x) and x.shape[0] >= TAPS_MIN_ROIS
+
+
+def _tap_call(name, *args):
+    rc = getattr(lib(), name)(*args, _stream())
+    if rc:
+        raise RuntimeError("%s failed (%d)" % (name, rc))
+
+
+def tap_gather(x, plan, in_pm, R):
+    C = x.shape[-1]
+    cols = torch.empty((plan.units * R * C,), dtype=torch.float32, device=x.device)
+    with torch.cuda.device(x.device):
+        _tap_call("wsplumb_tap_gather", _p(x), R, C, _p(plan.device_table(x.device)), plan.hnum, int(in_pm), _p(cols))
+    return cols
+
+
+def tap_col2im(dcols, plan, in_pm, R, C):
+    shape = (plan.h * plan.w * R, C) if in_pm else (R, plan.h, plan.w, C)
+    dx = torch.empty(shape, dtype=torch.float32, device=dcols.device)
+    with torch.cuda.device(dcols.device):
+        _tap_call("wsplumb_tap_col2im", _p(dcols), R, C, _p(plan.device_table(dcols.device)), plan.hnum, int(in_pm),
+                  _p(dx))
+    return dx
+
+
+def tap_weight_gather(weight, plan):
+    CO, C = weight.shape[0], weight.shape[1] // 9
+    wp = torch.empty((plan.wunits * CO * C,), dtype=torch.float32, device=weight.device)
+    with torch.cuda.device(weight.device):
+        _tap_call("wsplumb_tap_weight_gather", _p(weight), CO, C, _p(plan.device_table(weight.device)), plan.hnum,
+                  _p(wp))
+    return wp
+
+
+def tap_weight_scatter(dwp, plan, CO, C):
+    dw = torch.empty((CO, 9 * C), dtype=torch.float32, device=dwp.device)
+    with torch.cuda.device(dwp.device):
+        _tap_call("wsplumb_tap_weight_scatter", _p(dwp), CO, C, _p(plan.device_table(dwp.device)), plan.hnum, _p(dw))
+    return dw
+
+
+def _gemm_groups(plan, fn):
+    for k0, n, npos, ntaps in plan.groups:
+        if TAP_GEMM_GROUPED or n == 1:
+            fn(k0, n, npos, ntaps, slice(0, n))
+        else:
+            for j in range(n):
+                fn(k0, n, npos, ntaps, slice(j, j + 1))
+
+
+class TapConv3x3Fn(torch.autograd.Function):
+
+    @staticmethod
+    def forward(ctx, x, weight, bias, plan, in_pm, R):
+        C, CO = weight.shape[1] // 9, weight.shape[0]
+        x = x.contiguous()
+        assert x.shape[-1] == C and x.numel() == plan.h * plan.w * R * C and (not in_pm or plan.h == plan.oh)
+        cols = tap_gather(x, plan, in_pm, R)
+        wp = tap_weight_gather(weight.contiguous(), plan)
+        out = torch.empty((plan.oh * plan.ow * R, CO), dtype=torch.float32, device=x.device)
+
+        def gemm(k0, n, npos, ntaps, j):
+            a = cols[plan.cum[k0] * R * C:(plan.cum[k0] + n * npos * ntaps) * R * C].view(n, npos * R, ntaps * C)
+            b = wp[plan.wcum[k0] * CO * C:(plan.wcum[k0] + n * ntaps) * CO * C].view(n, CO, ntaps * C)
+            o = out[plan.slot_base[k0] * R:(plan.slot_base[k0] + n * npos) * R].view(n, npos * R, CO)
+            if j.stop - j.start == 1:
+                torch.mm(a[j.start], b[j.start].t(), out=o[j.start])
+            else:
+                torch.bmm(a, b.transpose(1, 2), out=o)
+
+        _gemm_groups(plan, gemm)
+        if bias is not None:
+            out.add_(bias)
+        ctx.save_for_backward(cols, wp)
+        ctx.geom = (plan, bool(in_pm), R, C, CO, bias is not None)
+        return out
+
+    @staticmethod
+    def backward(ctx, dy):
+        cols, wp = ctx.saved_tensors
+        plan, in_pm, R, C, CO, has_bias = ctx.geom
+        dy = dy.contiguous()
+        need_x, need_w = ctx.needs_input_grad[0], ctx.needs_input_grad[1]
+        dcols = torch.empty_like(cols) if need_x else None
+        dwp = torch.empty_like(wp) if need_w else None
+
+        def gemm(k0, n, npos, ntaps, j):
+            g = dy[plan.slot_base[k0] * R:(plan.slot_base[k0] + n * npos) * R].view(n, npos * R, CO)
+            cs = slice(plan.cum[k0] * R * C, (plan.cum[k0] + n * npos * ntaps) * R * C)
+            ws = slice(plan.wcum[k0] * CO * C, (plan.wcum[k0] + n * ntaps) * CO * C)
+            one = j.stop - j.start == 1
+            if need_x:
+                b = wp[ws].view(n, CO, ntaps * C)
+                o = dcols[cs].view(n, npos * R, ntaps * C)
+                if one:
+                    torch.mm(g[j.start], b[j.start], out=o[j.start])
+                else:
+                    torch.bmm(g, b, out=o)
+            if need_w:
+                a = cols[cs].view(n, npos * R, ntaps * C)
+                o = dwp[ws].view(n, CO, ntaps * C)
+                if one:
+                    torch.mm(g[j.start].t(), a[j.start], out=o[j.start])
+                else:
+                    torch.bmm(g.transpose(1, 2), a, out=o)
+
+        _gemm_groups(plan, gemm)
+        dx = tap_col2im(dcols, plan, in_pm, R, C) if need_x else None
+        dw = tap_weight_scatter(dwp, plan, CO, C) if need_w else None
+        db = None
+        if has_bias and ctx.needs_input_grad[2]:
+            db = dy.sum(0)
+        return dx, dw, db, None, None, None
diff --git a/wssdl_bus_amd/networks/roi_head.py b/wssdl_bus_amd/networks/roi_head.py
--- a/wssdl_bus_amd/networks/roi_head.py
+++ b/wssdl_bus_amd/networks/roi_head.py
@@ -36,9 +36,9 @@
 class _FusedRowBatchNormFn(torch.autograd.Function):
 
     @staticmethod
-    def forward(ctx, x, weight, bias, eps, relu, roi_mask=None):
-        y, stats, count = _plumbing.rowbn_forward(x, weight, bias, eps, relu, roi_mask)
-        ctx.masked = roi_mask is not None
+    def forward(ctx, x, weight, bias, eps, relu, roi_mask=None, pos_major=False):
+        y, stats, count = _plumbing.rowbn_forward(x, weight, bias, eps, relu, roi_mask, pos_major)
+        ctx.masked, ctx.pos_major = roi_mask is not None, pos_major
         if ctx.masked:
             ctx.save_for_backward(x, weight, stats, roi_mask)
         else:
@@ -55,8 +55,8 @@
             x, weight, stats, roi_mask = ctx.saved_tensors
         else:
             (x, weight, stats), roi_mask = ctx.saved_tensors, None
-        dx, dw, db = _plumbing.rowbn_backward(x, dy.contiguous(), weight, stats, ctx.relu, roi_mask)
-        return dx, dw, db, None, None, None
+        dx, dw, db = _plumbing.rowbn_backward(x, dy.contiguous(), weight, stats, ctx.relu, roi_mask, ctx.pos_major)
+        return dx, dw, db, None, None, None, None
 
 
 _ROI_MASK = None
@@ -67,10 +67,10 @@
     _ROI_MASK = mask
 
 
-def _masked_row_batch_norm(x, weight, bias, eps, relu, roi_mask):
+def _masked_row_batch_norm(x, weight, bias, eps, relu, roi_mask, pos_major=False):
     M = x.shape[0]
     per = M // roi_mask.shape[0]
-    m = roi_mask.repeat_interleave(per).unsqueeze(1)
+    m = (roi_mask.repeat(per) if pos_major else roi_mask.repeat_interleave(per)).unsqueeze(1)
     n = (roi_mask.sum() * per).clamp_min(1.0)
     mean = (x * m).sum(0) / n
     d = (x - mean) * m
@@ -91,7 +91,7 @@
         self.register_buffer("running_mean", torch.zeros(num_features))
         self.register_buffer("running_var", torch.ones(num_features))
 
-    def forward(self, x, relu=False):
+    def forward(self, x, relu=False, pos_major=False):
         fused = _plumbing.usable(x)
         if not self.training:
             scale = self.weight * torch.rsqrt(self.running_var + self.eps)
@@ -102,10 +102,12 @@
             return F.relu(y) if relu else y
         if _ROI_MASK is not None:
             if fused and x.shape[0] % _ROI_MASK.shape[0] == 0:
-                y, mean, var, n = _FusedRowBatchNormFn.apply(x, self.weight, self.bias, self.eps, bool(relu), _ROI_MASK)
+                y, mean, var, n = _FusedRowBatchNormFn.apply(x, self.weight, self.bias, self.eps, bool(relu), _ROI_MASK,
+                                                             bool(pos_major))
                 n = n[0]
             else:
-                y, mean, var, n = _masked_row_batch_norm(x, self.weight, self.bias, self.eps, relu, _ROI_MASK)
+                y, mean, var, n = _masked_row_batch_norm(x, self.weight, self.bias, self.eps, relu, _ROI_MASK,
+                                                         pos_major)
             with torch.no_grad():
                 self.running_mean.lerp_(mean, self.momentum)
                 self.running_var.lerp_(var * (n / (n - 1).clamp_min(1.0)), self.momentum)
@@ -153,12 +155,27 @@
             p = xp.unfold(1, k, s).unfold(2, k, s)
             oh, ow = p.shape[1], p.shape[2]
             rows = p.permute(0, 1, 2, 4, 5, 3).reshape(-1, k * k * c)
-        y = F.linear(rows, self.weight, self.bias)
+        return self._act(F.linear(rows, self.weight, self.bias)).view(r, oh, ow, self.c_o)
+
+    def _act(self, y, pos_major=False):
         if self.bn is not None:
-            y = self.bn(y, relu=self.relu)
-        elif self.relu:
-            y = F.relu(y)
-        return y.view(r, oh, ow, self.c_o)
+            return self.bn(y, relu=self.relu, pos_major=pos_major)
+        return F.relu(y) if self.relu else y
+
+    def forward_pm(self, x, plan, R):
+        if self.k == 3:
+            y = _plumbing.TapConv3x3Fn.apply(x, self.weight, self.bias, plan, x.dim() == 2, R)
+        else:
+            if x.dim() == 4:
+                x = _pm_rows(x, plan, self.s)
+            y = F.linear(x, self.weight, self.bias)
+        return self._act(y, pos_major=True)
+
+
+def _pm_rows(x, plan, s):
+    r, h, w, c = x.shape
+    idx = plan.subsample_index(w, s, x.device)
+    return x.view(r, h * w, c).transpose(0, 1).index_select(0, idx).reshape(-1, c)
 
 
 def _bn_rows(bn, x, relu=False):
@@ -188,6 +205,25 @@
         x = self.conv3(self.conv2(self.conv1(x)))
         return x + (self.short(ori) if self.short is not None else ori)
 
+    def forward_pm(self, x, plans, R):
+        pm = x.dim() == 2
+        ori = x
+        if self.preact != "no_preact":
+            y = _pre_act(self.pre_bn, x, pm)
+            if self.preact == "both_preact":
+                ori = y
+            x = y
+        s = self.conv2.s
+        plan = plans[s]
+        if not pm:
+            x = self.conv1(x)
+        else:
+            x = self.conv1.forward_pm(x, plan, R)
+        x = self.conv3.forward_pm(self.conv2.forward_pm(x, plan, R), plan, R)
+        if self.short is not None:
+            return x + self.short.forward_pm(ori, plan, R)
+        return x + (ori if pm else _pm_rows(ori, plan, s))
+
 
 class BasicBlockNHWC(nn.Module):
     expansion = 1
@@ -210,6 +246,27 @@
         x = self.conv2(self.conv1(x))
         return x + (self.short(ori) if self.short is not None else ori)
 
+    def forward_pm(self, x, plans, R):
+        pm = x.dim() == 2
+        ori = x
+        if self.preact != "no_preact":
+            y = _pre_act(self.pre_bn, x, pm)
+            if self.preact == "both_preact":
+                ori = y
+            x = y
+        s = self.conv1.s
+        plan = plans[s]
+        x = self.conv2.forward_pm(self.conv1.forward_pm(x, plan, R), plans[1], R)
+        if self.short is not None:
+            return x + self.short.forward_pm(ori, plan, R)
+        return x + (ori if pm else _pm_rows(ori, plan, s))
+
+
+def _pre_act(bn, x, pm):
+    if not pm:
+        return _bn_rows(bn, x, relu=True) if bn is not None else F.relu(x)
+    return bn(x, relu=True, pos_major=True) if bn is not None else F.relu(x)
+
 
 class ResNetHeadNHWC(nn.Module):
 
@@ -226,6 +283,26 @@
         self.out_features = 512 * e
 
     def forward(self, x):
+        plans = self._tap_plans(x)
+        if plans is not None:
+            return self._forward_pm(x, plans)
         x = self.group3(x)
         x = _bn_rows(self.norm, x, relu=True) if self.norm is not None else F.relu(x)
         return x.mean(dim=(1, 2))
+
+    @staticmethod
+    def _tap_plans(x):
+        if not _plumbing.taps_usable(x):
+            return None
+        p2 = _plumbing.tap_plan(x.shape[1], x.shape[2], 2)
+        p1 = _plumbing.tap_plan(p2.oh, p2.ow, 1)
+        if not (p2.ok and p1.ok and p1.slots == p2.slots):
+            return None
+        return {2: p2, 1: p1}
+
+    def _forward_pm(self, x, plans):
+        R = x.shape[0]
+        for blk in self.group3:
+            x = blk.forward_pm(x, plans, R)
+        x = self.norm(x, relu=True, pos_major=True) if self.norm is not None else F.relu(x)
+        return x.view(-1, R, x.shape[1]).mean(dim=0)
```

Result: faster. 51.82 images/s, median of 6 (+6.1%).
